# TrondVQ/UncertaintyQuantification-SleepApnea-1DCNN

Hardware: AMD Instinct MI355X
Metric: 30s-windows/sec for MCD T=50 & DE M=8 inference at 1/2/4/8 MI355X (higher is better)
Workload: dtype fp32; 1 GPU; global_batch=16384, seq_len=60, parallelism=dp1, mcd_passes=50, de_members=8, bn_mode_mcd=batch

## Files before the change

uncertaintyquantification_sleepapnea_1dcnn_amd/csrc/x3_args.h:

```cpp
#pragma once

namespace apneauq {
namespace x3 {

struct LayerArgs {
  const float* in;
  float* out;
  const void* wfrag;
  long long w_gstride;
  const float* bias;
  const float* wscale;
  int p_gstride;
  const float* aff_in;
  int aff_gstride;
  const unsigned* smax_in;
  const float* amax_in;
  unsigned* smax_out;
  const float* gscale_in;
  double* stats;
  int n_win;
  int groups;
  int tiles_per_group;
  int total_tiles;
  int in_shared;
  int sign_in;
  int sign_out;
  unsigned thr_in;
  unsigned thr_out;
  int layer;
  unsigned pass_base;
  unsigned window_offset;
  unsigned long long seed;
};

struct L1Args {
  const float* x;
  const float* w;
  const float* b;
  float* out;
  double* stats;
  unsigned* smax;
  int n_win, groups, blocks_per_group;
};

struct AffArgs {
  const double* stats;
  const float* gamma;
// ... 28 lines not shown
```

uncertaintyquantification_sleepapnea_1dcnn_amd/csrc/x3_bindings.cpp:

```cpp
#include <ATen/ATen.h>
#include <c10/core/DeviceGuard.h>
#include <c10/hip/HIPStream.h>
#include <torch/library.h>

#include <hip/hip_runtime_api.h>

#include "x3_args.h"

namespace apneauq {
int x3_lds_bytes(int layer);
int x3_tile_samples(int layer);
int x3_wg_per_cu(int layer);
hipError_t x3_launch_layer(int layer, const x3::LayerArgs& A, int grid, hipStream_t stream);
hipError_t x3_launch_l1(const x3::L1Args& A, hipStream_t stream);
hipError_t x3_launch_aff(const x3::AffArgs& A, hipStream_t stream);
hipError_t x3_launch_head(const x3::HeadArgs& A, hipStream_t stream);
}

namespace {

constexpr int kCh[7] = {4, 128, 192, 224, 96, 256, 96};
constexpr int kKs[6] = {7, 5, 3, 7, 9, 9};

inline hipStream_t cur_stream() { return c10::hip::getCurrentHIPStream().stream(); }
inline void check(hipError_t e, const char* what) { TORCH_CHECK(e == hipSuccess, what, " failed: ", hipGetErrorString(e)); }

inline void need(const at::Tensor& t, at::ScalarType dt, int64_t min_numel, const char* what) {
  TORCH_CHECK(t.is_cuda() && t.scalar_type() == dt && t.is_contiguous(), what, ": contiguous GPU tensor of dtype ", dt,
// ... 2 lines not shown
  TORCH_CHECK(reinterpret_cast<uintptr_t>(t.data_ptr()) % 16 == 0, what, ": 16-B alignment required");
}

int num_cus(const at::Tensor& t) {
  int n = 0;
  check(hipDeviceGetAttribute(&n, hipDeviceAttributeMultiprocessorCount, t.device().index()), "hipDeviceGetAttribute");
  return n > 0 ? n : 256;
}

void x3_layer(int64_t layer, const at::Tensor& in, at::Tensor& out, const at::Tensor& wfrag, int64_t w_gstride,
              const at::Tensor& bias, const at::Tensor& wscale, int64_t p_gstride, const at::Tensor& aff_in,
              int64_t aff_gstride, const c10::optional<at::Tensor>& stats, int64_t n_win, int64_t groups,
              bool in_shared, int64_t thr_in, int64_t thr_out, int64_t seed, int64_t pass_base,
              int64_t window_offset, int64_t grid, const c10::optional<at::Tensor>& smax_in,
              const c10::optional<at::Tensor>& amax_in, const c10::optional<at::Tensor>& smax_out,
              const c10::optional<at::Tensor>& gscale_in, bool sign_in, bool sign_out) {
  TORCH_CHECK(layer >= 1 && layer <= 5, "x3_layer: layer must be 1..5 (block 2..6)");
  TORCH_CHECK(n_win >= 1 && groups >= 1, "x3_layer: empty launch");
  const int cin = kCh[layer], cout = kCh[layer + 1], ks = kKs[layer];
  const int64_t samples = n_win * groups, samples_in = in_shared ? n_win : samples;
  const int ts = apneauq::x3_tile_samples((int)layer);
  const int64_t tpg = (n_win + ts - 1) / ts;
  TORCH_CHECK(tpg * groups < (int64_t(1) << 31), "x3_layer: too many tiles");
  const int64_t wgroups = w_gstride ? groups : 1, pgroups = p_gstride ? groups : 1;
  need(in, at::kFloat, samples_in * 60 * cin, "x3_layer: in");
  need(out, at::kFloat, layer == 5 ? samples * 2 * cout : samples * 60 * cout, "x3_layer: out");
  const int64_t frag = (int64_t)(cin / 32) * ks * (cout / 16) * 128;
  TORCH_CHECK(w_gstride == 0 || w_gstride == frag, "x3_layer: w_gstride must be 0 or ", frag);
  need(wfrag, at::kHalf, wgroups * frag * 8, "x3_layer: wfrag");
  TORCH_CHECK(p_gstride == 0 || p_gstride == cout, "x3_layer: p_gstride must be 0 or ", cout);
  need(bias, at::kFloat, pgroups * cout, "x3_layer: bias");
// ... 9 lines not shown
  const bool pre = smax_in.has_value() && smax_in->defined();
  TORCH_CHECK(pre == (amax_in.has_value() && amax_in->defined()), "x3_layer: smax_in and amax_in go together");
  if (pre) {
    need(*smax_in, at::kInt, samples_in, "x3_layer: smax_in");
    need(*amax_in, at::kFloat, (aff_gstride ? groups : 1) * 2, "x3_layer: amax_in");
  }
  const bool gpre = gscale_in.has_value() && gscale_in->defined();
  TORCH_CHECK(!(pre && gpre), "x3_layer: per-sample and per-group prescale are exclusive");
  if (gpre) need(*gscale_in, at::kFloat, aff_gstride ? groups : 1, "x3_layer: gscale_in");
  unsigned* smo = nullptr;
  if (smax_out.has_value() && smax_out->defined()) {
    TORCH_CHECK(layer < 5, "x3_layer: block 6 feeds the fp32 head (no smax_out)");
    need(*smax_out, at::kInt, samples, "x3_layer: smax_out");
    smo = reinterpret_cast<unsigned*>(smax_out->data_ptr<int>());
  }
  const at::DeviceGuard guard(in.device());
  apneauq::x3::LayerArgs A;
  A.in = in.data_ptr<float>();
  A.out = out.data_ptr<float>();
  A.wfrag = wfrag.data_ptr();
  A.w_gstride = w_gstride;
  A.bias = bias.data_ptr<float>();
  A.wscale = wscale.data_ptr<float>();
  A.p_gstride = (int)p_gstride;
  A.aff_in = aff_in.data_ptr<float>();
  A.aff_gstride = (int)aff_gstride;
  A.stats = st;
  A.smax_in = pre ? reinterpret_cast<const unsigned*>(smax_in->data_ptr<int>()) : nullptr;
  A.amax_in = pre ? amax_in->data_ptr<float>() : nullptr;
  A.smax_out = smo;
  A.gscale_in = gpre ? gscale_in->data_ptr<float>() : nullptr;
  A.n_win = (int)n_win;
// ... 1 lines not shown
  A.tiles_per_group = (int)tpg;
  A.total_tiles = (int)(tpg * groups);
  A.in_shared = in_shared ? 1 : 0;
  TORCH_CHECK(!(sign_in && in_shared), "x3_layer: the shared block-1 output carries no masks");
  TORCH_CHECK(!(sign_out && layer == 5), "x3_layer: block 6 reduces its masked output in place");
  A.sign_in = sign_in ? 1 : 0;
  A.sign_out = sign_out ? 1 : 0;
  A.thr_in = (unsigned)thr_in;
  A.thr_out = (unsigned)thr_out;
  A.layer = (int)layer;
  A.pass_base = (unsigned)pass_base;
  A.window_offset = (unsigned)window_offset;
  A.seed = (unsigned long long)seed;
  int g = grid > 0 ? (int)grid : num_cus(in) * apneauq::x3_wg_per_cu((int)layer);
  if (g > A.total_tiles) g = A.total_tiles;
  check(apneauq::x3_launch_layer((int)layer, A, g, cur_stream()), "x3_layer");
}

void x3_l1(const at::Tensor& x, const at::Tensor& w, const at::Tensor& b, at::Tensor& out,
           const c10::optional<at::Tensor>& stats, int64_t n_win, int64_t groups, const c10::optional<at::Tensor>& smax) {
  TORCH_CHECK(n_win >= 1 && groups >= 1, "x3_l1: empty launch");
  need(x, at::kFloat, n_win * 60 * 4, "x3_l1: x");
  need(w, at::kFloat, groups * 7 * 4 * 128, "x3_l1: w");
  need(b, at::kFloat, groups * 128, "x3_l1: b");
  need(out, at::kFloat, groups * n_win * 60 * 128, "x3_l1: out");
  double* st = nullptr;
  if (stats.has_value()) {
    need(*stats, at::kDouble, groups * apneauq::x3::kStatSlots * 2 * 128, "x3_l1: stats");
    st = stats->data_ptr<double>();
  }
  unsigned* smp = nullptr;
// ... 55 lines not shown
  TORCH_CHECK(aff_gstride == 0 || aff_gstride == 2 * C, "x3_head: aff_gstride");
  TORCH_CHECK(p_gstride == 0 || p_gstride == C, "x3_head: p_gstride");
  need(sums, at::kFloat, samples * 2 * C, "x3_head: sums");
  need(aff, at::kFloat, (aff_gstride ? groups : 1) * 2 * C, "x3_head: aff");
  need(dw, at::kFloat, (p_gstride ? groups : 1) * C, "x3_head: dense w");
  need(db, at::kFloat, p_gstride ? groups : 1, "x3_head: dense b");
  need(out, at::kFloat, samples, "x3_head: out");
  const at::DeviceGuard guard(sums.device());
  apneauq::x3::HeadArgs A{sums.data_ptr<float>(), aff.data_ptr<float>(), dw.data_ptr<float>(), db.data_ptr<float>(),
                          out.data_ptr<float>(), C, (int)n_win, (int)samples, (int)aff_gstride, (int)p_gstride,
                          logits ? 1 : 0};
  check(apneauq::x3_launch_head(A, cur_stream()), "x3_head");
}

int64_t x3_lds(int64_t layer) { return apneauq::x3_lds_bytes((int)layer); }

}

TORCH_LIBRARY_FRAGMENT(apneauq, m) {
  m.def("x3_layer(int layer, Tensor input, Tensor(a!) out, Tensor wfrag, int w_gstride, Tensor bias, Tensor wscale, "
        "int p_gstride, Tensor aff_in, int aff_gstride, Tensor(b!)? stats, int n_win, int groups, bool in_shared, "
        "int thr_in, int thr_out, int seed, int pass_base, int window_offset, int grid, Tensor? smax_in=None, "
        "Tensor? amax_in=None, Tensor(c!)? smax_out=None, Tensor? gscale_in=None, bool sign_in=False, bool sign_out=False) -> ()");
  m.def("x3_l1(Tensor x, Tensor w, Tensor b, Tensor(a!) out, Tensor(b!)? stats, int n_win, int groups, "
        "Tensor(c!)? smax=None) -> ()");
  m.def("x3_aff(Tensor? stats, Tensor gamma, Tensor beta, Tensor(a!) mmean, Tensor(b!) mvar, Tensor(c!) aff, int C, "
        "int groups, int p_gstride, bool update, int repeat, float inv_count, float eps, float momentum, float dsc, "
        "Tensor(d!)? amax=None, Tensor(e!)? gscale=None, bool running=False) -> ()");
  m.def("x3_head(Tensor sums, Tensor aff, int aff_gstride, Tensor dw, Tensor db, int p_gstride, Tensor(a!) out, "
        "int n_win, int groups, bool logits) -> ()");
  m.def("x3_lds(int layer) -> int", &x3_lds);
}

TORCH_LIBRARY_IMPL(apneauq, CUDA, m) {
  m.impl("x3_layer", &x3_layer);
  m.impl("x3_l1", &x3_l1);
  m.impl("x3_head", &x3_head);
  m.impl("x3_aff", &x3_aff);
}
```

uncertaintyquantification_sleepapnea_1dcnn_amd/csrc/x3_layers.hip:

```cpp
#include "common.h"
#include "x3_args.h"

namespace apneauq {
namespace x3 {

typedef _Float16 f16x8 __attribute__((ext_vector_type(8)));
typedef _Float16 f16x4 __attribute__((ext_vector_type(4)));
typedef _Float16 f16x2 __attribute__((ext_vector_type(2)));
typedef __attribute__((address_space(1))) const f16x8 gf16x8;

constexpr int kStagers = 4;
constexpr int kL = 60, kSR = 64, kHalo = 4;
__host__ __device__ constexpr int row_bytes(int ck) { return 4 * ck + 32; }
__device__ __forceinline__ int sample_prescale(unsigned rmax_bits, const float* amax) {
  const float b = __builtin_fmaf(amax[0], __uint_as_float(rmax_bits), amax[1]);
  int e = 0;
  if (b > 0.f && b < INFINITY) frexpf(b, &e);
  return min(100, max(-100, 14 - e));
}

__host__ __device__ constexpr int lds_rows(int S) { return kHalo + S * kSR + kHalo; }
__host__ __device__ constexpr int buf_bytes(int S, int ck) { return lds_rows(S) * row_bytes(ck); }
__host__ __device__ constexpr int lds_bytes(int S, int cout, int ck) {
  return 2 * buf_bytes(S, ck) + 2 * cout * 8 + 2 * S * 4;
}

template <typename T>
__device__ __forceinline__ T gld(const void* p) {
  return *(const __attribute__((address_space(1))) T*)(p);
}

__device__ __forceinline__ int opaque_tid() {
  int t = threadIdx.x;
  asm volatile("" : "+v"(t));
  return t;
}

__device__ __forceinline__ f32x4 mfma(const f16x8& a, const f16x8& b, const f32x4& c) {
  return __builtin_amdgcn_mfma_f32_16x16x32_f16(a, b, c, 0, 0, 0);
// ... 2 lines not shown
__device__ __forceinline__ void lds_barrier() {
  __builtin_amdgcn_fence(__ATOMIC_RELEASE, "workgroup", "local");
  __builtin_amdgcn_s_barrier();
  __builtin_amdgcn_fence(__ATOMIC_ACQUIRE, "workgroup", "local");
}

__device__ __forceinline__ int xcd_wg() {
  const int nwg = gridDim.x, bid = blockIdx.x;
  const int q = nwg / 8, rem = nwg % 8, xcd = bid % 8;
  return (xcd < rem ? xcd * (q + 1) : rem * (q + 1) + (xcd - rem) * q) + bid / 8;
}

template <int NW, int WPC>
constexpr int waves_per_eu() { return NW * WPC > 8 ? (NW * WPC + 3) / 4 : NW * WPC <= 4 ? 1 : 2; }
constexpr int loaders(int lw) { return lw > 0 ? lw : 0; }
template <int CIN, int COUT, int KS, int S, int WM, int WN, bool LAST, int LW, int CK, int WPC, bool PS>
__global__ __launch_bounds__((WM * WN + loaders(LW)) * 64, (waves_per_eu<WM * WN + loaders(LW), WPC>())) void layer_kernel(
    const LayerArgs A) {
  extern __shared__ __attribute__((aligned(16))) char smem[];
  constexpr int NWM = WM * WN, NW = NWM + loaders(LW), kThreads = NW * 64;
  constexpr int kCK = CK, kRowB = row_bytes(CK), NQ = CK / 32, kQ = CK / 4;
  constexpr int kS = S, kBufB = buf_bytes(S, CK), kValidRows = S * kL, kUnits = kValidRows * kQ;
  constexpr int SW = LW > 0 ? LW : LW < 0 ? (-LW < NW ? -LW : NW) : (kStagers < NW ? kStagers : NW);
  constexpr int kSBase = LW > 0 ? NWM * 64 : 0;
  constexpr int kST = SW * 64;
  constexpr int kNU = (kUnits + kST - 1) / kST;
  static_assert(kST % kQ == 0 && (CK == 32 || CK == 64), "a staging thread keeps one channel quad");
  constexpr int NCH = CIN / kCK, NCTA = COUT / 16, NCT = NCTA / WN, NRT = 4 * S / WM, PAD = (KS - 1) / 2;
  constexpr int NSTEP = NCH * NQ * KS;
  constexpr int RG = NCT >= 4                        ? 1
                     : (NCT >= 3 && NCT * NRT > 16)    ? 1
                     : NCT == 1                        ? 4
                                                       : 2;
  constexpr bool BDB = NCT * NRT <= 24 && RG < 4;
  static_assert(NRT % RG == 0, "row-tile groups");
  constexpr long long FRAG_STEP = (long long)NCTA * 128;
  static_assert(CIN % kCK == 0 && COUT % 16 == 0, "channel tiling");
  static_assert(NCTA % WN == 0 && (4 * S) % WM == 0, "wave tiling");
  static_assert(NRT % 4 == 0, "whole 64-row sample slots per wave row (epilogue keys, block 6 sums)");
  double* st = reinterpret_cast<double*>(smem + 2 * kBufB);
  float* wsc = reinterpret_cast<float*>(smem + 2 * kBufB + 2 * COUT * 8);

  const int tid = threadIdx.x, lane = tid & 63;
  const int wave = __builtin_amdgcn_readfirstlane(tid >> 6);
  const int wn = wave % WN, wm = (wave / WN) % WM;
  const int ct0 = wn * NCT, rt0 = wm * NRT;
  const int m = lane & 15, h = lane >> 4;
  APNEAUQ_DASSERT(blockDim.x == kThreads);

  for (int i = tid; i < 2 * kBufB / 16; i += kThreads) reinterpret_cast<f32x4*>(smem)[i] = f32x4{0.f, 0.f, 0.f, 0.f};
  for (int i = tid; i < 2 * COUT; i += kThreads) st[i] = 0.0;
  __syncthreads();

  const int wg = xcd_wg();
  const int tpg = (A.n_win + S - 1) / S;
  const int total_tiles = tpg * A.groups;
  const int t_begin = (int)((long long)wg * total_tiles / gridDim.x);
  const int t_end = (int)((long long)(wg + 1) * total_tiles / gridDim.x);
  if (t_begin >= t_end) return;
  const int slot = wg % kStatSlots;

  const bool loader = LW > 0 && wave >= NWM;
  const bool stager = LW > 0 ? loader : wave < SW;
  struct Stage {
    f32x4 v[kNU];
    f32x4 a, b;
// ... 292 lines not shown
  auto flush_stats = [&](int g) {
    __syncthreads();
    if (A.stats != nullptr) {
      double* dst = A.stats + ((long long)g * kStatSlots + slot) * 2 * COUT;
      for (int i = tid; i < 2 * COUT; i += kThreads) {
        atomicAdd(dst + i, st[i]);
        st[i] = 0.0;
      }
    }
    __syncthreads();
  };

  const int total = (t_end - t_begin) * NCH;
  auto chunk_tile = [&](int it) { return t_begin + it / NCH; };
  int g_cur = t_begin / tpg;
  if constexpr (LW > 0) {
    if (loader) {
      if (stager) {
        load_chunk(t_begin, 0, s0);
        store_chunk(t_begin, 0, smem, s0);
      }
      lds_barrier();
      if (stager && total > 1) load_chunk(chunk_tile(1), 1 % NCH, s0);
#pragma unroll 1
      for (int it = 0; it < total; ++it) {
        const int tile = chunk_tile(it), c = it - (tile - t_begin) * NCH;
        if (c == 0) {
          const int g = tile / tpg;
          if (g != g_cur) {
            flush_stats(g_cur);
// ... 206 lines not shown
  const long long sidx = (long long)blockIdx.x * 4 + (threadIdx.x >> 6);
  if (sidx >= A.samples) return;
  const int g = (int)(sidx / A.n_win);
  const float* s = A.sums + sidx * 2 * A.C;
  const float* af = A.aff + (long long)g * A.aff_gstride;
  const float* dw = A.dw + (long long)g * A.p_gstride;
  float v = 0.f;
  for (int c = lane; c < A.C; c += 64) v += dw[c] * __builtin_fmaf(af[c], s[c], af[A.C + c] * s[A.C + c]);
  v = wave_sum(v);
  if (lane == 0) {
    const float logit = v * (1.0f / kL) + A.db[A.p_gstride ? g : 0];
    A.out[sidx] = A.out_logits ? logit : 1.0f / (1.0f + expf(-logit));
  }
}

template <int CIN, int COUT, int KS, int S, int WM, int WN, bool LAST, int LW, int CK, int WPC, bool PS>
hipError_t launch_layer(const LayerArgs& A, int grid, hipStream_t stream) {
  constexpr int lds = lds_bytes(S, COUT, CK);
  static_assert(WPC * lds <= 160 * 1024, "LDS of the workgroups sharing a CU");
  auto k = layer_kernel<CIN, COUT, KS, S, WM, WN, LAST, LW, CK, WPC, PS>;
  static bool attr = false;
  if (!attr) {
    hipError_t e = hipFuncSetAttribute(reinterpret_cast<const void*>(k), hipFuncAttributeMaxDynamicSharedMemorySize, lds);
    if (e != hipSuccess) return e;
    attr = true;
  }
  hipLaunchKernelGGL(k, dim3(grid), dim3((WM * WN + loaders(LW)) * 64), lds, stream, A);
  return hipGetLastError();
}

}

#ifdef APNEAUQ_X3_TABLE
#include APNEAUQ_X3_TABLE
#else
#define APNEAUQ_X3_LAYERS(X)                     \
  X(1, 128, 192, 5, 4, 2, 4, false, -8, 0, 32, 1) \
  X(2, 192, 224, 3, 2, 1, 7, false, 4, 4, 64, 1) \
  X(3, 224, 96, 7, 4, 2, 2, false, 4, 4, 32, 1)  \
  X(4, 96, 256, 9, 2, 1, 8, false, 4, 4, 32, 1)  \
  X(5, 256, 96, 9, 4, 2, 2, true, 4, 4, 64, 1)
#endif

int x3_lds_bytes(int layer) {
#define APNEAUQ_X3_LDS(L, CI, CO, K, S, WM, WN, LAST, LW, LWB, CK, WPC) \
  if (layer == L) return x3::lds_bytes(S, CO, CK);
  APNEAUQ_X3_LAYERS(APNEAUQ_X3_LDS)
#undef APNEAUQ_X3_LDS
  return 0;
}

int x3_tile_samples(int layer) {
#define APNEAUQ_X3_TS(L, CI, CO, K, S, WM, WN, LAST, LW, LWB, CK, WPC) \
  if (layer == L) return S;
  APNEAUQ_X3_LAYERS(APNEAUQ_X3_TS)
#undef APNEAUQ_X3_TS
  return 0;
}

int x3_wg_per_cu(int layer) {
#define APNEAUQ_X3_WPC(L, CI, CO, K, S, WM, WN, LAST, LW, LWB, CK, WPC) \
  if (layer == L) return WPC;
  APNEAUQ_X3_LAYERS(APNEAUQ_X3_WPC)
#undef APNEAUQ_X3_WPC
  return 1;
}

hipError_t x3_launch_layer(int layer, const x3::LayerArgs& A, int grid, hipStream_t stream) {
  using namespace x3;
  const bool ps = A.smax_in != nullptr || A.smax_out != nullptr;
#define APNEAUQ_X3_LAUNCH(L, CI, CO, K, S, WM, WN, LAST, LW, LWB, CK, WPC)                                  \
  if (layer == L) {                                                                                       \
    return ps ? launch_layer<CI, CO, K, S, WM, WN, LAST, LW, CK, WPC, true>(A, grid, stream)               \
              : launch_layer<CI, CO, K, S, WM, WN, LAST, LWB, CK, WPC, false>(A, grid, stream);            \
  }
  APNEAUQ_X3_LAYERS(APNEAUQ_X3_LAUNCH)
#undef APNEAUQ_X3_LAUNCH
  return hipErrorInvalidValue;
}

hipError_t x3_launch_l1(const x3::L1Args& A, hipStream_t stream) {
  const int grid = A.groups * A.blocks_per_group;
  if (grid <= 0) return hipSuccess;
  hipLaunchKernelGGL(x3::l1_kernel, dim3(grid), dim3(256), 0, stream, A);
  return hipGetLastError();
}

hipError_t x3_launch_aff(const x3::AffArgs& A, hipStream_t stream) {
  const int blocks = A.groups + (A.stats != nullptr && A.update ? 1 : 0);
// ... 12 lines not shown
```

uncertaintyquantification_sleepapnea_1dcnn_amd/ops/x3.py:

```python
from __future__ import annotations

import math
import os
from typing import Callable, Dict, List, Optional, Sequence

import torch

from ..models.spec import ModelSpec
from . import _ext, fused, rng

CH = fused.FUSED_CHANNELS
KS = fused.FUSED_KSIZES
STAT_SLOTS = 16
TILE = 4
CK = 32
BYTES_PER_SAMPLE = 60 * (192 + 256) * 4
R1_BYTES = 60 * 128 * 4


def supports(spec: ModelSpec) -> bool:
    return fused.supports(spec)


def pack_conv(kernel: torch.Tensor):
# ... 74 lines not shown

class _Workspace:
    def __init__(self, dev, samples: int, n_r1: int, groups: int):
        self.samples, self.n_r1, self.groups = int(samples), int(n_r1), max(int(groups), 1)
        f32 = dict(dtype=torch.float32, device=dev)
        self.r1 = torch.empty(n_r1 * 60 * CH[1], **f32)
        self.buf = [torch.empty(samples * 60 * 192, **f32), torch.empty(samples * 60 * 256, **f32)]
        self.sums = torch.empty(samples * 2 * CH[6], **f32)
        self.out = torch.empty(samples, **f32)
        self.stats = [torch.zeros(max(groups, 1) * STAT_SLOTS * 2 * CH[l + 1], dtype=torch.float64, device=dev)
                      for l in range(6)]
        self.aff = [torch.empty(max(groups, 1) * 2 * CH[l + 1], **f32) for l in range(6)]
        self.smax = [torch.zeros(n_r1 if l == 0 else samples, dtype=torch.int32, device=dev) for l in range(5)]
        self.amax = [torch.zeros(max(groups, 1) * 2, **f32) for l in range(6)]
        self.gscale = [torch.ones(max(groups, 1), **f32) for l in range(5)] + [None]

    def smax_out(self, l: int, k: int) -> Optional[torch.Tensor]:
        if l >= 5:
            return None
        return self.smax[l][:k].zero_()


def _ops():
    return _ext.ops()


_SIGN_DEFAULT = "2,4"


def _sign_layers() -> frozenset:
    v = os.environ.get("APNEAUQ_X3_SIGN_MASK", _SIGN_DEFAULT)
    return frozenset(int(t) for t in v.replace(" ", "").split(",") if t)


def _sign(l: int, sl: frozenset):
    return (l - 1) in sl and l >= 2, l in sl and l <= 4


def _dsc(rate: float) -> float:
    return 1.0 / (1.0 - rate) if rate < 1.0 else 0.0


def _sync_stats(sync: Callable, st: torch.Tensor, groups: int, c: int) -> None:
    v = st[: groups * STAT_SLOTS * 2 * c].view(groups, STAT_SLOTS, 2 * c)
    tot = v.sum(1)
    sync(tot)
    v.zero_()
    v[:, 0].copy_(tot)


def _max_samples(dev, per_sample: int, frac: float = 0.45) -> int:
# ... 30 lines not shown
        w = dist.get_world_size() if dist.is_initialized() else 1
        ref_n = -(-gn // w)
    if ref_n > max_samples:
        return _mcd_batch_windowed(model, x, n_pass, seed, pass_base, window_offset, update_moving, sync, gn,
                                   max_samples)
    cap = max(1, min(n_pass, max_samples // max(ref_n, 1)))
    n_chunks = -(-n_pass // cap)
    chunk = -(-n_pass // n_chunks)
    ws = model.workspace(chunk * n, n, chunk)
    inv_count = 1.0 / (gn * 60.0)
    thr = [rng.dropout_threshold(b.dropout) for b in spec.blocks]
    dsc = [_dsc(b.dropout) for b in spec.blocks]
    eps, mom = float(spec.bn_epsilon), float(spec.bn_momentum)
    seed = int(seed) & ((1 << 63) - 1)
    sl = _sign_layers()
    out = torch.empty(n_pass, n, dtype=torch.float32, device=model.device)
    ws.stats[0].zero_()
    o.x3_l1(x, model.w1, model.b1, ws.r1, ws.stats[0], n, 1, None)
    if sync is not None:
        _sync_stats(sync, ws.stats[0], 1, CH[1])
    g, b, mm, mv = model.bn[0]
    o.x3_aff(ws.stats[0], g, b, mm, mv, ws.aff[0], CH[1], 1, 0, bool(update_moving), n_pass, inv_count, eps, mom, dsc[0],
             None, ws.gscale[0])
    for t0 in range(0, n_pass, chunk):
        tc = min(chunk, n_pass - t0)
        pb = int(pass_base) + t0
        for l in range(1, 6):
            c = CH[l + 1]
            st = ws.stats[l]
            st[: tc * STAT_SLOTS * 2 * c].zero_()
            src = ws.r1 if l == 1 else ws.buf[(l - 2) % 2]
            dst = ws.sums if l == 5 else ws.buf[(l - 1) % 2]
            o.x3_layer(l, src, dst, model.wfrag[l], 0, model.bias[l], model.wscale[l], 0, ws.aff[l - 1],
                       0 if l == 1 else 2 * CH[l], st, n, tc, l == 1, thr[l - 1], thr[l], seed, pb,
                       int(window_offset), int(grid), None, None, None, ws.gscale[l - 1], *_sign(l, sl))
            if sync is not None:
                _sync_stats(sync, st, tc, c)
            g, b, mm, mv = model.bn[l]
            o.x3_aff(st, g, b, mm, mv, ws.aff[l], c, tc, 0, bool(update_moving), 1, inv_count, eps, mom, dsc[l],
                     None, ws.gscale[l])
        o.x3_head(ws.sums, ws.aff[5], 2 * CH[6], model.dw, model.db, 0, ws.out, n, tc, False)
        out[t0: t0 + tc].copy_(ws.out[: tc * n].view(tc, n))
    return out


def _mcd_batch_windowed(model: X3Model, x: torch.Tensor, n_pass: int, seed: int, pass_base: int,
                        window_offset: int, update_moving: bool, sync: Optional[Callable], gn: int,
                        max_samples: int) -> torch.Tensor:
    spec, o = model.spec, _ops()
    n = x.shape[0]
    wc = max(1, int(max_samples))
    bounds = [(s, min(n, s + wc)) for s in range(0, n, wc)]
    ws = model.workspace(wc, wc, 1)
    inv_count = 1.0 / (gn * 60.0)
    thr = [rng.dropout_threshold(b.dropout) for b in spec.blocks]
    dsc = [_dsc(b.dropout) for b in spec.blocks]
    eps, mom = float(spec.bn_epsilon), float(spec.bn_momentum)
    seed = int(seed) & ((1 << 63) - 1)
    sl = _sign_layers()
    out = torch.empty(n_pass, n, dtype=torch.float32, device=model.device)

    def run(s: int, e: int, upto: int, pb: int, stats_layer: int) -> None:
        m = e - s
        o.x3_l1(x[s:e], model.w1, model.b1, ws.r1, ws.stats[0] if stats_layer == 0 else None, m, 1, None)
        for l in range(1, upto + 1):
            src = ws.r1 if l == 1 else ws.buf[(l - 2) % 2]
            dst = ws.sums if l == 5 else ws.buf[(l - 1) % 2]
            o.x3_layer(l, src, dst, model.wfrag[l], 0, model.bias[l], model.wscale[l], 0, ws.aff[l - 1],
                       0 if l == 1 else 2 * CH[l], ws.stats[l] if l == stats_layer else None, m, 1, l == 1,
                       thr[l - 1], thr[l], seed, pb, int(window_offset) + s, 0, None, None, None, ws.gscale[l - 1],
                       *_sign(l, sl))

    def finish_layer(l: int, repeat: int) -> None:
        if sync is not None:
            _sync_stats(sync, ws.stats[l], 1, CH[l + 1])
        g, b, mm, mv = model.bn[l]
        o.x3_aff(ws.stats[l], g, b, mm, mv, ws.aff[l], CH[l + 1], 1, 0, bool(update_moving), repeat, inv_count, eps,
                 mom, dsc[l], None, ws.gscale[l])

    ws.stats[0].zero_()
    for s, e in bounds:
        run(s, e, 0, int(pass_base), 0)
    finish_layer(0, n_pass)
    for t in range(n_pass):
        pb = int(pass_base) + t
        for l in range(1, 6):
            ws.stats[l].zero_()
            for s, e in bounds:
                run(s, e, l, pb, l)
            finish_layer(l, 1)
        for s, e in bounds:
            run(s, e, 5, pb, -1)
            o.x3_head(ws.sums, ws.aff[5], 0, model.dw, model.db, 0, ws.out, e - s, 1, False)
            out[t, s:e].copy_(ws.out[: e - s])
    return out


@torch.no_grad()
def forward_running(model: X3Model, x: torch.Tensor, n_pass: int = 1, dropout: bool = False, seed: int = 0,
                    pass_offset: int = 0, window_offset: int = 0, logits: bool = False,
                    max_samples: Optional[int] = None) -> torch.Tensor:
    x = x.to(device=model.device, dtype=torch.float32).contiguous()
    n = x.shape[0]
    groups = (n_pass if dropout else model.G) if n > 0 else 1
    if max_samples is None:
        max_samples = _max_samples(model.device, BYTES_PER_SAMPLE + R1_BYTES)
    wc = max(1, int(max_samples) // max(groups, 1))
    if n <= wc:
        return _forward_running(model, x, n_pass, dropout, seed, pass_offset, window_offset, logits)
# ... 8 lines not shown
    n = x.shape[0]
    G = model.G
    if dropout and G != 1:
        raise ValueError("MC Dropout runs one model")
    if not dropout:
        n_pass = 1
    groups = n_pass if dropout else G
    ws = model.workspace(groups * n, n * G, max(groups, G))
    thr = [rng.dropout_threshold(b.dropout) if dropout else 0 for b in spec.blocks]
    dsc = [_dsc(b.dropout) if dropout else 1.0 for b in spec.blocks]
    eps, mom = float(spec.bn_epsilon), float(spec.bn_momentum)
    seed = int(seed) & ((1 << 63) - 1)
    if not dropout:
        return _predict_members(model, ws, x, G, eps, mom, logits)
    sl = _sign_layers()
    for l in range(6):
        g, b, mm, mv = model.bn[l]
        o.x3_aff(None, g, b, mm, mv, ws.aff[l], CH[l + 1], G, CH[l + 1] if G > 1 else 0, False, 1, 1.0, eps, mom,
                 dsc[l], ws.amax[l])
    o.x3_l1(x, model.w1, model.b1, ws.r1, None, n, G, ws.smax[0])
    per_member = G > 1
    for l in range(1, 6):
        src = ws.r1 if l == 1 else ws.buf[(l - 2) % 2]
        dst = ws.sums if l == 5 else ws.buf[(l - 1) % 2]
        wstride = model.wfrag[l].shape[1] // 8 if per_member else 0
        sm = ws.smax_out(l, groups * n)
        o.x3_layer(l, src, dst, model.wfrag[l], wstride, model.bias[l], model.wscale[l],
                   CH[l + 1] if per_member else 0, ws.aff[l - 1], 2 * CH[l] if per_member else 0, None, n, groups,
                   dropout and l == 1, thr[l - 1], thr[l], seed, int(pass_offset),
                   int(window_offset), 0, ws.smax[l - 1], ws.amax[l - 1], sm, None, *_sign(l, sl))
    o.x3_head(ws.sums, ws.aff[5], 2 * CH[6] if per_member else 0, model.dw, model.db, CH[6] if per_member else 0,
              ws.out, n, groups, bool(logits))
    return ws.out[: groups * n].view(G, n_pass, n).clone()


def _predict_members(model: X3Model, ws: "_Workspace", x: torch.Tensor, G: int, eps: float, mom: float,
                     logits: bool) -> torch.Tensor:
    spec, o = model.spec, _ops()
    n = x.shape[0]
    per_member = G > 1
    ps = CH[1:] if per_member else [0] * 6
    o.zero_buffers([ws.stats[l][: G * STAT_SLOTS * 2 * CH[l + 1]] for l in range(5)])
    g, b, mm, mv = model.bn[5]
    o.x3_aff(None, g, b, mm, mv, ws.aff[5], CH[6], G, ps[5], False, 1, 1.0, eps, mom, 1.0, None)
    o.x3_l1(x, model.w1, model.b1, ws.r1, ws.stats[0], n, G, None)
    for l in range(1, 6):
        g, b, mm, mv = model.bn[l - 1]
        o.x3_aff(ws.stats[l - 1], g, b, mm, mv, ws.aff[l - 1], CH[l], G, ps[l - 1], False, 1, 1.0, eps, mom, 1.0,
                 None, ws.gscale[l - 1], True)
        src = ws.r1 if l == 1 else ws.buf[(l - 2) % 2]
        dst = ws.sums if l == 5 else ws.buf[(l - 1) % 2]
        wstride = model.wfrag[l].shape[1] // 8 if per_member else 0
        o.x3_layer(l, src, dst, model.wfrag[l], wstride, model.bias[l], model.wscale[l], ps[l],
                   ws.aff[l - 1], 2 * CH[l] if per_member else 0, ws.stats[l] if l < 5 else None, n, G, False, 0, 0,
                   0, 0, 0, 0, None, None, None, ws.gscale[l - 1], False, False)
    o.x3_head(ws.sums, ws.aff[5], 2 * CH[6] if per_member else 0, model.dw, model.db, CH[6] if per_member else 0,
              ws.out, n, G, bool(logits))
    return ws.out[: G * n].view(G, 1, n).clone()


def split_f16(a: torch.Tensor):
    hi = a.half()
    lo = (a - hi.float()).half()
    return hi, lo


def emulate_conv(h: torch.Tensor, fr: torch.Tensor, wscale: float, k: int, cin: int, cout: int) -> torch.Tensor:
    from ..models.reference import conv1d_same

    nch, nct = cin // CK, cout // 16
    v = fr.reshape(nch, k, nct, 2, 4, 16, 8).double()
    whi = v[:, :, :, 0].permute(1, 0, 3, 5, 2, 4).reshape(k, cin, cout)
# ... 7 lines not shown
```

Baseline: 63270 windows/s.

## Add LDS chunk ring with counter-based producer/consumer sync for layer 4

Replaces the double-buffered, barrier-synchronised chunk staging with a configurable-depth LDS ring. Loader or stager waves and compute waves coordinate through per-slot full/empty atomic counters instead of workgroup barriers, and only block 5 (layer 4) is enabled with depth 3. The goal is to let loads run further ahead of the MFMA compute and to cut barrier stalls. In exchange it uses more LDS, adds spin-waits with bounded timeouts that poison the outputs and set an error word, and keeps an environment switch to turn the ring off.

Result: no change. 63450 windows/s (median of 3 runs) (+0.3%).

```diff
diff --git a/uncertaintyquantification_sleepapnea_1dcnn_amd/csrc/x3_args.h b/uncertaintyquantification_sleepapnea_1dcnn_amd/csrc/x3_args.h
--- a/uncertaintyquantification_sleepapnea_1dcnn_amd/csrc/x3_args.h
+++ b/uncertaintyquantification_sleepapnea_1dcnn_amd/csrc/x3_args.h
@@ -31,6 +31,7 @@
   unsigned pass_base;
   unsigned window_offset;
   unsigned long long seed;
+  unsigned* err;
 };
 
 struct L1Args {
diff --git a/uncertaintyquantification_sleepapnea_1dcnn_amd/csrc/x3_bindings.cpp b/uncertaintyquantification_sleepapnea_1dcnn_amd/csrc/x3_bindings.cpp
--- a/uncertaintyquantification_sleepapnea_1dcnn_amd/csrc/x3_bindings.cpp
+++ b/uncertaintyquantification_sleepapnea_1dcnn_amd/csrc/x3_bindings.cpp
@@ -11,7 +11,8 @@
 int x3_lds_bytes(int layer);
 int x3_tile_samples(int layer);
 int x3_wg_per_cu(int layer);
-hipError_t x3_launch_layer(int layer, const x3::LayerArgs& A, int grid, hipStream_t stream);
+int x3_ring_depth(int layer);
+hipError_t x3_launch_layer(int layer, const x3::LayerArgs& A, int grid, hipStream_t stream, bool ring);
 hipError_t x3_launch_l1(const x3::L1Args& A, hipStream_t stream);
 hipError_t x3_launch_aff(const x3::AffArgs& A, hipStream_t stream);
 hipError_t x3_launch_head(const x3::HeadArgs& A, hipStream_t stream);
@@ -44,7 +45,8 @@
               bool in_shared, int64_t thr_in, int64_t thr_out, int64_t seed, int64_t pass_base,
               int64_t window_offset, int64_t grid, const c10::optional<at::Tensor>& smax_in,
               const c10::optional<at::Tensor>& amax_in, const c10::optional<at::Tensor>& smax_out,
-              const c10::optional<at::Tensor>& gscale_in, bool sign_in, bool sign_out) {
+              const c10::optional<at::Tensor>& gscale_in, bool sign_in, bool sign_out,
+              const c10::optional<at::Tensor>& err, bool ring) {
   TORCH_CHECK(layer >= 1 && layer <= 5, "x3_layer: layer must be 1..5 (block 2..6)");
   TORCH_CHECK(n_win >= 1 && groups >= 1, "x3_layer: empty launch");
   const int cin = kCh[layer], cout = kCh[layer + 1], ks = kKs[layer];
@@ -84,8 +86,14 @@
     need(*smax_out, at::kInt, samples, "x3_layer: smax_out");
     smo = reinterpret_cast<unsigned*>(smax_out->data_ptr<int>());
   }
+  unsigned* errp = nullptr;
+  if (err.has_value() && err->defined()) {
+    need(*err, at::kInt, 1, "x3_layer: err");
+    errp = reinterpret_cast<unsigned*>(err->data_ptr<int>());
+  }
   const at::DeviceGuard guard(in.device());
   apneauq::x3::LayerArgs A;
+  A.err = errp;
   A.in = in.data_ptr<float>();
   A.out = out.data_ptr<float>();
   A.wfrag = wfrag.data_ptr();
@@ -117,7 +125,7 @@
   A.seed = (unsigned long long)seed;
   int g = grid > 0 ? (int)grid : num_cus(in) * apneauq::x3_wg_per_cu((int)layer);
   if (g > A.total_tiles) g = A.total_tiles;
-  check(apneauq::x3_launch_layer((int)layer, A, g, cur_stream()), "x3_layer");
+  check(apneauq::x3_launch_layer((int)layer, A, g, cur_stream(), ring), "x3_layer");
 }
 
 void x3_l1(const at::Tensor& x, const at::Tensor& w, const at::Tensor& b, at::Tensor& out,
@@ -203,6 +211,7 @@
 }
 
 int64_t x3_lds(int64_t layer) { return apneauq::x3_lds_bytes((int)layer); }
+int64_t x3_ring_depth(int64_t layer) { return apneauq::x3_ring_depth((int)layer); }
 
 }
 
@@ -210,7 +219,8 @@
   m.def("x3_layer(int layer, Tensor input, Tensor(a!) out, Tensor wfrag, int w_gstride, Tensor bias, Tensor wscale, "
         "int p_gstride, Tensor aff_in, int aff_gstride, Tensor(b!)? stats, int n_win, int groups, bool in_shared, "
         "int thr_in, int thr_out, int seed, int pass_base, int window_offset, int grid, Tensor? smax_in=None, "
-        "Tensor? amax_in=None, Tensor(c!)? smax_out=None, Tensor? gscale_in=None, bool sign_in=False, bool sign_out=False) -> ()");
+        "Tensor? amax_in=None, Tensor(c!)? smax_out=None, Tensor? gscale_in=None, bool sign_in=False, bool sign_out=False, "
+        "Tensor(d!)? err=None, bool ring=True) -> ()");
   m.def("x3_l1(Tensor x, Tensor w, Tensor b, Tensor(a!) out, Tensor(b!)? stats, int n_win, int groups, "
         "Tensor(c!)? smax=None) -> ()");
   m.def("x3_aff(Tensor? stats, Tensor gamma, Tensor beta, Tensor(a!) mmean, Tensor(b!) mvar, Tensor(c!) aff, int C, "
@@ -219,6 +229,7 @@
   m.def("x3_head(Tensor sums, Tensor aff, int aff_gstride, Tensor dw, Tensor db, int p_gstride, Tensor(a!) out, "
         "int n_win, int groups, bool logits) -> ()");
   m.def("x3_lds(int layer) -> int", &x3_lds);
+  m.def("x3_ring_depth(int layer) -> int", &x3_ring_depth);
 }
 
 TORCH_LIBRARY_IMPL(apneauq, CUDA, m) {
diff --git a/uncertaintyquantification_sleepapnea_1dcnn_amd/csrc/x3_layers.hip b/uncertaintyquantification_sleepapnea_1dcnn_amd/csrc/x3_layers.hip
--- a/uncertaintyquantification_sleepapnea_1dcnn_amd/csrc/x3_layers.hip
+++ b/uncertaintyquantification_sleepapnea_1dcnn_amd/csrc/x3_layers.hip
@@ -1,5 +1,7 @@
 #include "common.h"
 #include "x3_args.h"
+#include "x3_ring.h"
+#include "x3_table.h"
 
 namespace apneauq {
 namespace x3 {
@@ -21,8 +23,9 @@
 
 __host__ __device__ constexpr int lds_rows(int S) { return kHalo + S * kSR + kHalo; }
 __host__ __device__ constexpr int buf_bytes(int S, int ck) { return lds_rows(S) * row_bytes(ck); }
-__host__ __device__ constexpr int lds_bytes(int S, int cout, int ck) {
-  return 2 * buf_bytes(S, ck) + 2 * cout * 8 + 2 * S * 4;
+__host__ __device__ constexpr int ring_bufs(int D) { return D > 0 ? D : 2; }
+__host__ __device__ constexpr int lds_bytes(int S, int cout, int ck, int D) {
+  return ring_bufs(D) * buf_bytes(S, ck) + 2 * cout * 8 + 2 * S * 4 + (D > 0 ? ((2 * D + 1) * 4 + 15) / 16 * 16 : 0);
 }
 
 template <typename T>
@@ -55,7 +58,7 @@
 template <int NW, int WPC>
 constexpr int waves_per_eu() { return NW * WPC > 8 ? (NW * WPC + 3) / 4 : NW * WPC <= 4 ? 1 : 2; }
 constexpr int loaders(int lw) { return lw > 0 ? lw : 0; }
-template <int CIN, int COUT, int KS, int S, int WM, int WN, bool LAST, int LW, int CK, int WPC, bool PS>
+template <int CIN, int COUT, int KS, int S, int WM, int WN, bool LAST, int LW, int CK, int WPC, bool PS, int D>
 __global__ __launch_bounds__((WM * WN + loaders(LW)) * 64, (waves_per_eu<WM * WN + loaders(LW), WPC>())) void layer_kernel(
     const LayerArgs A) {
   extern __shared__ __attribute__((aligned(16))) char smem[];
@@ -79,8 +82,14 @@
   static_assert(CIN % kCK == 0 && COUT % 16 == 0, "channel tiling");
   static_assert(NCTA % WN == 0 && (4 * S) % WM == 0, "wave tiling");
   static_assert(NRT % 4 == 0, "whole 64-row sample slots per wave row (epilogue keys, block 6 sums)");
-  double* st = reinterpret_cast<double*>(smem + 2 * kBufB);
-  float* wsc = reinterpret_cast<float*>(smem + 2 * kBufB + 2 * COUT * 8);
+  constexpr int NB = ring_bufs(D);
+  static_assert(ring::depth_ok(D, NCH), "ring depth: 0, or 2 <= D <= NCH (x3_ring.h, drift invariant of wsc[tile & 1])");
+  static_assert(SW == ring::staging_waves(LW, NW) && loaders(LW) == ring::loader_waves(LW), "x3_ring.h mirrors the staging layout");
+  double* st = reinterpret_cast<double*>(smem + NB * kBufB);
+  float* wsc = reinterpret_cast<float*>(smem + NB * kBufB + 2 * COUT * 8);
+  unsigned* rfull = reinterpret_cast<unsigned*>(smem + NB * kBufB + 2 * COUT * 8 + 2 * S * 4);
+  unsigned* rempty = rfull + NB;
+  unsigned* rabort = rempty + NB;
 
   const int tid = threadIdx.x, lane = tid & 63;
   const int wave = __builtin_amdgcn_readfirstlane(tid >> 6);
@@ -89,8 +98,11 @@
   const int m = lane & 15, h = lane >> 4;
   APNEAUQ_DASSERT(blockDim.x == kThreads);
 
-  for (int i = tid; i < 2 * kBufB / 16; i += kThreads) reinterpret_cast<f32x4*>(smem)[i] = f32x4{0.f, 0.f, 0.f, 0.f};
+  for (int i = tid; i < NB * kBufB / 16; i += kThreads) reinterpret_cast<f32x4*>(smem)[i] = f32x4{0.f, 0.f, 0.f, 0.f};
   for (int i = tid; i < 2 * COUT; i += kThreads) st[i] = 0.0;
+  if constexpr (D > 0) {
+    if (tid < 2 * D + 1) rfull[tid] = 0u;
+  }
   __syncthreads();
 
   const int wg = xcd_wg();
@@ -413,6 +425,135 @@
   const int total = (t_end - t_begin) * NCH;
   auto chunk_tile = [&](int it) { return t_begin + it / NCH; };
   int g_cur = t_begin / tpg;
+
+  if constexpr (D > 0) {
+    auto ring_peek = [&](const unsigned* ctr) -> unsigned {
+      unsigned v = 0u;
+      if (lane == 0) v = __hip_atomic_load(ctr, __ATOMIC_RELAXED, __HIP_MEMORY_SCOPE_WORKGROUP);
+      return v;
+    };
+    auto ring_wait = [&](const unsigned* ctr, unsigned need, unsigned seen, unsigned code) -> bool {
+      unsigned v = __builtin_amdgcn_readfirstlane(seen);
+      for (unsigned spins = 1u; !ring::reached(v, need); ++spins) {
+        unsigned why = spins > ring::kPollBudget ? code : 0u;
+        if (why == 0u && (spins & ring::kAbortCheckMask) == 0u && __builtin_amdgcn_readfirstlane(ring_peek(rabort)) != 0u)
+          why = ring::kErrAborted;
+        if (why != 0u) {
+          if (lane == 0) {
+            __hip_atomic_store(rabort, 1u, __ATOMIC_RELAXED, __HIP_MEMORY_SCOPE_WORKGROUP);
+            if (A.err != nullptr) atomicOr(A.err, why);
+          }
+          return false;
+        }
+        __builtin_amdgcn_s_sleep(1);
+        v = __builtin_amdgcn_readfirstlane(ring_peek(ctr));
+      }
+      __builtin_amdgcn_fence(__ATOMIC_ACQUIRE, "workgroup", "local");
+      return true;
+    };
+    auto ring_signal = [&](unsigned* ctr) {
+      __builtin_amdgcn_fence(__ATOMIC_RELEASE, "workgroup", "local");
+      if (lane == 0) __hip_atomic_fetch_add(ctr, 1u, __ATOMIC_RELAXED, __HIP_MEMORY_SCOPE_WORKGROUP);
+    };
+    auto poison = [&](int tile) {
+      const float qn = __builtin_nanf("");
+      const f32x4 q4 = {qn, qn, qn, qn};
+#pragma unroll 1
+      for (; tile < t_end; ++tile) {
+        const int g = tile / tpg, w0 = (tile - g * tpg) * kS;
+#pragma unroll 1
+        for (int i = 0; i < NCT * NRT; ++i) {
+          const int ct = i / NRT, rt = i - ct * NRT, co0 = (ct0 + ct) * 16 + 4 * h;
+          const int s = (rt0 + rt) >> 2, t = (((rt0 + rt) & 3) << 4) + m, w = w0 + s;
+          if (w >= A.n_win) continue;
+          const long long sample = (long long)g * A.n_win + w;
+          if constexpr (!LAST) {
+            if (t < kL) *reinterpret_cast<f32x4*>(A.out + (sample * kL + t) * COUT + co0) = q4;
+          } else if (m == 0 && (rt & 3) == 3) {
+            *reinterpret_cast<f32x4*>(A.out + sample * (2 * COUT) + co0) = q4;
+            *reinterpret_cast<f32x4*>(A.out + sample * (2 * COUT) + COUT + co0) = q4;
+          }
+        }
+      }
+    };
+    ring::Cursor cur{0, 0u};
+    if (loader) {
+      load_chunk(t_begin, 0, s0);
+#pragma unroll 1
+      for (int it = 0; it < total; ++it) {
+        const int tile = chunk_tile(it), c = it - (tile - t_begin) * NCH;
+        if (c == 0) {
+          const int g = tile / tpg;
+          if (g != g_cur) {
+            flush_stats(g_cur);
+            g_cur = g;
+          }
+        }
+        if (!ring_wait(rempty + cur.b, ring::empty_need(cur.n, NWM), ring_peek(rempty + cur.b), ring::kErrProducerTimeout))
+          return;
+        store_chunk(tile, c, smem + cur.b * kBufB, s0);
+        ring_signal(rfull + cur.b);
+        if (it + 1 < total) load_chunk(chunk_tile(it + 1), (it + 1) % NCH, s0);
+        cur = ring::next(cur, D);
+      }
+      flush_stats(g_cur);
+      return;
+    }
+    if (LW <= 0 && stager) {
+      load_chunk(t_begin, 0, s0);
+      store_chunk(t_begin, 0, smem, s0);
+      ring_signal(rfull);
+      if (total > 1) load_chunk(chunk_tile(1), 1 % NCH, s0);
+    }
+    unsigned seen = ring_peek(rfull);
+    load_a(wbase(t_begin), ah, al);
+    bool dead = false;
+    int tile = t_begin;
+#pragma unroll 1
+    for (int it = 0; it < total; ++it) {
+      tile = chunk_tile(it);
+      const int c = it - (tile - t_begin) * NCH;
+      if (c == 0) {
+        const int g = tile / tpg;
+        if (g != g_cur) {
+          flush_stats(g_cur);
+          g_cur = g;
+        }
+      }
+      if (!ring_wait(rfull + cur.b, ring::full_need(cur.n, SW), seen, ring::kErrConsumerTimeout)) {
+        dead = true;
+        break;
+      }
+      const ring::Cursor nx = ring::next(cur, D);
+      const gf16x8* wcur = wbase(tile);
+      const gf16x8* wnxt = wbase(tile + 1 < t_end ? tile + 1 : tile);
+      unsigned eseen = 0u;
+      if (LW <= 0 && stager) eseen = ring_peek(rempty + nx.b);
+      compute_chunk(c, smem + cur.b * kBufB, wcur, wnxt, [&]() {
+        if (LW <= 0 && stager && it + 1 < total) {
+          if (ring_wait(rempty + nx.b, ring::empty_need(nx.n, NWM), eseen, ring::kErrProducerTimeout)) {
+            store_chunk(chunk_tile(it + 1), (it + 1) % NCH, smem + nx.b * kBufB, s0);
+            ring_signal(rfull + nx.b);
+          } else {
+            dead = true;
+          }
+        }
+        seen = ring_peek(rfull + nx.b);
+      });
+      if (dead) break;
+      ring_signal(rempty + cur.b);
+      if (c == NCH - 1) epilogue(tile);
+      if (LW <= 0 && stager && it + 2 < total) load_chunk(chunk_tile(it + 2), (it + 2) % NCH, s0);
+      cur = nx;
+    }
+    if (dead) {
+      poison(tile);
+      return;
+    }
+    flush_stats(g_cur);
+    return;
+  }
+
   if constexpr (LW > 0) {
     if (loader) {
       if (stager) {
@@ -649,11 +790,11 @@
   }
 }
 
-template <int CIN, int COUT, int KS, int S, int WM, int WN, bool LAST, int LW, int CK, int WPC, bool PS>
+template <int CIN, int COUT, int KS, int S, int WM, int WN, bool LAST, int LW, int CK, int WPC, bool PS, int D>
 hipError_t launch_layer(const LayerArgs& A, int grid, hipStream_t stream) {
-  constexpr int lds = lds_bytes(S, COUT, CK);
+  constexpr int lds = lds_bytes(S, COUT, CK, D);
   static_assert(WPC * lds <= 160 * 1024, "LDS of the workgroups sharing a CU");
-  auto k = layer_kernel<CIN, COUT, KS, S, WM, WN, LAST, LW, CK, WPC, PS>;
+  auto k = layer_kernel<CIN, COUT, KS, S, WM, WN, LAST, LW, CK, WPC, PS, D>;
   static bool attr = false;
   if (!attr) {
     hipError_t e = hipFuncSetAttribute(reinterpret_cast<const void*>(k), hipFuncAttributeMaxDynamicSharedMemorySize, lds);
@@ -666,27 +807,17 @@
 
 }
 
-#ifdef APNEAUQ_X3_TABLE
-#include APNEAUQ_X3_TABLE
-#else
-#define APNEAUQ_X3_LAYERS(X)                     \
-  X(1, 128, 192, 5, 4, 2, 4, false, -8, 0, 32, 1) \
-  X(2, 192, 224, 3, 2, 1, 7, false, 4, 4, 64, 1) \
-  X(3, 224, 96, 7, 4, 2, 2, false, 4, 4, 32, 1)  \
-  X(4, 96, 256, 9, 2, 1, 8, false, 4, 4, 32, 1)  \
-  X(5, 256, 96, 9, 4, 2, 2, true, 4, 4, 64, 1)
-#endif
 
 int x3_lds_bytes(int layer) {
-#define APNEAUQ_X3_LDS(L, CI, CO, K, S, WM, WN, LAST, LW, LWB, CK, WPC) \
-  if (layer == L) return x3::lds_bytes(S, CO, CK);
+#define APNEAUQ_X3_LDS(L, CI, CO, K, S, WM, WN, LAST, LW, LWB, CK, WPC, D) \
+  if (layer == L) return x3::lds_bytes(S, CO, CK, D);
   APNEAUQ_X3_LAYERS(APNEAUQ_X3_LDS)
 #undef APNEAUQ_X3_LDS
   return 0;
 }
 
 int x3_tile_samples(int layer) {
-#define APNEAUQ_X3_TS(L, CI, CO, K, S, WM, WN, LAST, LW, LWB, CK, WPC) \
+#define APNEAUQ_X3_TS(L, CI, CO, K, S, WM, WN, LAST, LW, LWB, CK, WPC, D) \
   if (layer == L) return S;
   APNEAUQ_X3_LAYERS(APNEAUQ_X3_TS)
 #undef APNEAUQ_X3_TS
@@ -694,20 +825,31 @@
 }
 
 int x3_wg_per_cu(int layer) {
-#define APNEAUQ_X3_WPC(L, CI, CO, K, S, WM, WN, LAST, LW, LWB, CK, WPC) \
+#define APNEAUQ_X3_WPC(L, CI, CO, K, S, WM, WN, LAST, LW, LWB, CK, WPC, D) \
   if (layer == L) return WPC;
   APNEAUQ_X3_LAYERS(APNEAUQ_X3_WPC)
 #undef APNEAUQ_X3_WPC
   return 1;
 }
 
-hipError_t x3_launch_layer(int layer, const x3::LayerArgs& A, int grid, hipStream_t stream) {
+int x3_ring_depth(int layer) {
+#define APNEAUQ_X3_RD(L, CI, CO, K, S, WM, WN, LAST, LW, LWB, CK, WPC, D) \
+  if (layer == L) return D;
+  APNEAUQ_X3_LAYERS(APNEAUQ_X3_RD)
+#undef APNEAUQ_X3_RD
+  return 0;
+}
+
+hipError_t x3_launch_layer(int layer, const x3::LayerArgs& A, int grid, hipStream_t stream, bool ring) {
   using namespace x3;
   const bool ps = A.smax_in != nullptr || A.smax_out != nullptr;
-#define APNEAUQ_X3_LAUNCH(L, CI, CO, K, S, WM, WN, LAST, LW, LWB, CK, WPC)                                  \
+#define APNEAUQ_X3_LAUNCH(L, CI, CO, K, S, WM, WN, LAST, LW, LWB, CK, WPC, D)                                \
   if (layer == L) {                                                                                       \
-    return ps ? launch_layer<CI, CO, K, S, WM, WN, LAST, LW, CK, WPC, true>(A, grid, stream)               \
-              : launch_layer<CI, CO, K, S, WM, WN, LAST, LWB, CK, WPC, false>(A, grid, stream);            \
+    if (ring && D > 0)                                                                                    \
+      return ps ? launch_layer<CI, CO, K, S, WM, WN, LAST, LW, CK, WPC, true, D>(A, grid, stream)          \
+                : launch_layer<CI, CO, K, S, WM, WN, LAST, LWB, CK, WPC, false, D>(A, grid, stream);       \
+    return ps ? launch_layer<CI, CO, K, S, WM, WN, LAST, LW, CK, WPC, true, 0>(A, grid, stream)            \
+              : launch_layer<CI, CO, K, S, WM, WN, LAST, LWB, CK, WPC, false, 0>(A, grid, stream);         \
   }
   APNEAUQ_X3_LAYERS(APNEAUQ_X3_LAUNCH)
 #undef APNEAUQ_X3_LAUNCH
diff --git a/uncertaintyquantification_sleepapnea_1dcnn_amd/csrc/x3_ring.h b/uncertaintyquantification_sleepapnea_1dcnn_amd/csrc/x3_ring.h
--- /dev/null
+++ b/uncertaintyquantification_sleepapnea_1dcnn_amd/csrc/x3_ring.h
@@ -0,0 +1,41 @@
+#pragma once
+
+#if defined(__HIPCC__) || defined(__CUDACC__)
+#define APNEAUQ_RING_HD __host__ __device__
+#else
+#define APNEAUQ_RING_HD
+#endif
+
+namespace apneauq {
+namespace x3 {
+namespace ring {
+
+struct Cursor {
+  int b;
+  unsigned n;
+};
+APNEAUQ_RING_HD constexpr Cursor cursor_at(long long it, int D) { return Cursor{(int)(it % D), (unsigned)(it / D)}; }
+APNEAUQ_RING_HD constexpr Cursor next(Cursor c, int D) {
+  return c.b + 1 == D ? Cursor{0, c.n + 1u} : Cursor{c.b + 1, c.n};
+}
+APNEAUQ_RING_HD constexpr unsigned full_need(unsigned n, int SW) { return (unsigned)SW * (n + 1u); }
+APNEAUQ_RING_HD constexpr unsigned empty_need(unsigned n, int NWM) { return (unsigned)NWM * n; }
+APNEAUQ_RING_HD constexpr bool reached(unsigned counter, unsigned need) { return (int)(counter - need) >= 0; }
+
+APNEAUQ_RING_HD constexpr int loader_waves(int lw) { return lw > 0 ? lw : 0; }
+APNEAUQ_RING_HD constexpr int staging_waves(int lw, int nwm) {
+  return lw > 0 ? lw : lw < 0 ? (-lw < nwm ? -lw : nwm) : (4 < nwm ? 4 : nwm);
+}
+
+APNEAUQ_RING_HD constexpr bool depth_ok(int D, int NCH) { return D == 0 || (D >= 2 && D <= NCH); }
+
+constexpr unsigned kPollBudget = 1u << 22;
+constexpr unsigned kAbortCheckMask = 255u;
+
+constexpr unsigned kErrConsumerTimeout = 1u;
+constexpr unsigned kErrProducerTimeout = 2u;
+constexpr unsigned kErrAborted = 4u;
+
+}
+}
+}
diff --git a/uncertaintyquantification_sleepapnea_1dcnn_amd/csrc/x3_table.h b/uncertaintyquantification_sleepapnea_1dcnn_amd/csrc/x3_table.h
--- /dev/null
+++ b/uncertaintyquantification_sleepapnea_1dcnn_amd/csrc/x3_table.h
@@ -0,0 +1,12 @@
+#pragma once
+
+#ifdef APNEAUQ_X3_TABLE
+#include APNEAUQ_X3_TABLE
+#else
+#define APNEAUQ_X3_LAYERS(X)                        \
+  X(1, 128, 192, 5, 4, 2, 4, false, -8, 0, 32, 1, 0) \
+  X(2, 192, 224, 3, 2, 1, 7, false, 4, 4, 64, 1, 0) \
+  X(3, 224, 96, 7, 4, 2, 2, false, 4, 4, 32, 1, 0)  \
+  X(4, 96, 256, 9, 2, 1, 8, false, 4, 4, 32, 1, 3)  \
+  X(5, 256, 96, 9, 4, 2, 2, true, 4, 4, 64, 1, 0)
+#endif
diff --git a/uncertaintyquantification_sleepapnea_1dcnn_amd/ops/x3.py b/uncertaintyquantification_sleepapnea_1dcnn_amd/ops/x3.py
--- a/uncertaintyquantification_sleepapnea_1dcnn_amd/ops/x3.py
+++ b/uncertaintyquantification_sleepapnea_1dcnn_amd/ops/x3.py
@@ -112,6 +112,7 @@
         self.smax = [torch.zeros(n_r1 if l == 0 else samples, dtype=torch.int32, device=dev) for l in range(5)]
         self.amax = [torch.zeros(max(groups, 1) * 2, **f32) for l in range(6)]
         self.gscale = [torch.ones(max(groups, 1), **f32) for l in range(5)] + [None]
+        self.err = torch.zeros(1, dtype=torch.int32, device=dev)
 
     def smax_out(self, l: int, k: int) -> Optional[torch.Tensor]:
         if l >= 5:
@@ -133,6 +134,27 @@
 
 def _sign(l: int, sl: frozenset):
     return (l - 1) in sl and l >= 2, l in sl and l <= 4
+
+
+def _ring() -> bool:
+    return os.environ.get("APNEAUQ_X3_RING", "1") not in ("0", "")
+
+
+def ring_error(model: "X3Model", clear: bool = False) -> int:
+    ws = model._ws.get("ws")
+    if ws is None:
+        return 0
+    v = int(ws.err.item())
+    if clear:
+        ws.err.zero_()
+    return v
+
+
+def _check_ring(model: "X3Model") -> None:
+    if os.environ.get("APNEAUQ_X3_CHECK", "0") not in ("0", ""):
+        v = ring_error(model)
+        if v:
+            raise RuntimeError(f"x3 chunk ring: a bounded spin ran out (error word {v:#x}); the outputs are poisoned")
 
 
 def _dsc(rate: float) -> float:
@@ -193,6 +215,7 @@
     eps, mom = float(spec.bn_epsilon), float(spec.bn_momentum)
     seed = int(seed) & ((1 << 63) - 1)
     sl = _sign_layers()
+    ring = _ring()
     out = torch.empty(n_pass, n, dtype=torch.float32, device=model.device)
     ws.stats[0].zero_()
     o.x3_l1(x, model.w1, model.b1, ws.r1, ws.stats[0], n, 1, None)
@@ -212,7 +235,7 @@
             dst = ws.sums if l == 5 else ws.buf[(l - 1) % 2]
             o.x3_layer(l, src, dst, model.wfrag[l], 0, model.bias[l], model.wscale[l], 0, ws.aff[l - 1],
                        0 if l == 1 else 2 * CH[l], st, n, tc, l == 1, thr[l - 1], thr[l], seed, pb,
-                       int(window_offset), int(grid), None, None, None, ws.gscale[l - 1], *_sign(l, sl))
+                       int(window_offset), int(grid), None, None, None, ws.gscale[l - 1], *_sign(l, sl), ws.err, ring)
             if sync is not None:
                 _sync_stats(sync, st, tc, c)
             g, b, mm, mv = model.bn[l]
@@ -220,6 +243,7 @@
                      None, ws.gscale[l])
         o.x3_head(ws.sums, ws.aff[5], 2 * CH[6], model.dw, model.db, 0, ws.out, n, tc, False)
         out[t0: t0 + tc].copy_(ws.out[: tc * n].view(tc, n))
+    _check_ring(model)
     return out
 
 
@@ -237,6 +261,7 @@
     eps, mom = float(spec.bn_epsilon), float(spec.bn_momentum)
     seed = int(seed) & ((1 << 63) - 1)
     sl = _sign_layers()
+    ring = _ring()
     out = torch.empty(n_pass, n, dtype=torch.float32, device=model.device)
 
     def run(s: int, e: int, upto: int, pb: int, stats_layer: int) -> None:
@@ -248,7 +273,7 @@
             o.x3_layer(l, src, dst, model.wfrag[l], 0, model.bias[l], model.wscale[l], 0, ws.aff[l - 1],
                        0 if l == 1 else 2 * CH[l], ws.stats[l] if l == stats_layer else None, m, 1, l == 1,
                        thr[l - 1], thr[l], seed, pb, int(window_offset) + s, 0, None, None, None, ws.gscale[l - 1],
-                       *_sign(l, sl))
+                       *_sign(l, sl), ws.err, ring)
 
     def finish_layer(l: int, repeat: int) -> None:
         if sync is not None:
@@ -272,6 +297,7 @@
             run(s, e, 5, pb, -1)
             o.x3_head(ws.sums, ws.aff[5], 0, model.dw, model.db, 0, ws.out, e - s, 1, False)
             out[t, s:e].copy_(ws.out[: e - s])
+    _check_ring(model)
     return out
 
 
@@ -310,6 +336,7 @@
     if not dropout:
         return _predict_members(model, ws, x, G, eps, mom, logits)
     sl = _sign_layers()
+    ring = _ring()
     for l in range(6):
         g, b, mm, mv = model.bn[l]
         o.x3_aff(None, g, b, mm, mv, ws.aff[l], CH[l + 1], G, CH[l + 1] if G > 1 else 0, False, 1, 1.0, eps, mom,
@@ -324,9 +351,10 @@
         o.x3_layer(l, src, dst, model.wfrag[l], wstride, model.bias[l], model.wscale[l],
                    CH[l + 1] if per_member else 0, ws.aff[l - 1], 2 * CH[l] if per_member else 0, None, n, groups,
                    dropout and l == 1, thr[l - 1], thr[l], seed, int(pass_offset),
-                   int(window_offset), 0, ws.smax[l - 1], ws.amax[l - 1], sm, None, *_sign(l, sl))
+                   int(window_offset), 0, ws.smax[l - 1], ws.amax[l - 1], sm, None, *_sign(l, sl), ws.err, ring)
     o.x3_head(ws.sums, ws.aff[5], 2 * CH[6] if per_member else 0, model.dw, model.db, CH[6] if per_member else 0,
               ws.out, n, groups, bool(logits))
+    _check_ring(model)
     return ws.out[: groups * n].view(G, n_pass, n).clone()
 
 
@@ -335,6 +363,7 @@
     spec, o = model.spec, _ops()
     n = x.shape[0]
     per_member = G > 1
+    ring = _ring()
     ps = CH[1:] if per_member else [0] * 6
     o.zero_buffers([ws.stats[l][: G * STAT_SLOTS * 2 * CH[l + 1]] for l in range(5)])
     g, b, mm, mv = model.bn[5]
@@ -349,9 +378,10 @@
         wstride = model.wfrag[l].shape[1] // 8 if per_member else 0
         o.x3_layer(l, src, dst, model.wfrag[l], wstride, model.bias[l], model.wscale[l], ps[l],
                    ws.aff[l - 1], 2 * CH[l] if per_member else 0, ws.stats[l] if l < 5 else None, n, G, False, 0, 0,
-                   0, 0, 0, 0, None, None, None, ws.gscale[l - 1], False, False)
+                   0, 0, 0, 0, None, None, None, ws.gscale[l - 1], False, False, ws.err, ring)
     o.x3_head(ws.sums, ws.aff[5], 2 * CH[6] if per_member else 0, model.dw, model.db, CH[6] if per_member else 0,
               ws.out, n, G, bool(logits))
+    _check_ring(model)
     return ws.out[: G * n].view(G, 1, n).clone()
 
 
```
